# uc-vision/torch-darktable

Hardware: AMD Instinct MI355X
Metric: megapixels/sec full ISP (debayer->denoise->tonemap) 12MP RGGB (higher is better)
Workload: dtype f32; 1 GPU; 12 MP full pipeline (RCD -> Wiener log-L sigma=0.075 K=32 ov=4 -> bilateral sigma_s=2 sigma_r=0.2 detail=0.4 -> metrics -> Reinhard gamma=0.75 intensity=2 light_adapt=1 -> u8), batch 8 per GPU; width=4096, height=3072, streams_per_gpu=3, storage=f16, arithmetic=f32, chain=lab, issue=eager launches, denoiser=Wiener (the reference has no nlmeans / wavelet denoiser)

## Files before the change

### torch-darktable_amd/csrc/bilateral.hip

```cpp
#include <stdlib.h>

#include "tdk_color.h"

#ifdef TDK_BIL_TIMING
__device__ unsigned long long g_bil_phase_cycles[16];
#define BIL_MARK(k) do { if (threadIdx.x == 0 && blockIdx.x == 1000) { const unsigned long long t_ = clock64(); atomicAdd(&g_bil_phase_cycles[k], t_ - bil_t0); bil_t0 = t_; } } while (0)
extern "C" __attribute__((visibility("default"))) int tdk_debug_bilateral_phase_cycles(unsigned long long* out16, int reset) {
  if (hipMemcpyFromSymbol(out16, HIP_SYMBOL(g_bil_phase_cycles), sizeof(unsigned long long) * 16) != hipSuccess) return -1;
  if (reset) { unsigned long long z[16] = {}; if (hipMemcpyToSymbol(HIP_SYMBOL(g_bil_phase_cycles), z, sizeof z) != hipSuccess) return -1; }
  return 0;
}
#else
#define BIL_MARK(k)
#endif

namespace {

struct GridDims {
  int sx, sy, sz;
};

GridDims compute_grid_size(int width, int height, float sigma_s, float sigma_r) {
  float ss = sigma_s;
  if (ss < 0.5f) ss = 0.5f;
  const float L_range = 1.0f;
  auto clampf_h = [](float v, float lo, float hi) { return fminf(fmaxf(v, lo), hi); };
  const float gx = clampf_h(roundf((float)width / ss), 4.0f, 3000.0f);
  const float gy = clampf_h(roundf((float)height / ss), 4.0f, 3000.0f);
  const float gz = clampf_h(roundf(L_range / sigma_r), 4.0f, 50.0f);
  const float s_s = fmaxf((float)height / gy, (float)width / gx);
  const float s_r = L_range / gz;
  GridDims d;
  d.sx = (int)ceilf((float)width / s_s) + 1;
  d.sy = (int)ceilf((float)height / s_s) + 1;
  d.sz = (int)ceilf(L_range / s_r) + 1;
  return d;
}

struct Sample {
  int ix, iy, iz;
  float fx, fy, fz;
};

__device__ __forceinline__ Sample make_sample(int x, int y, float L, GridDims d, float sigma_s, float sigma_r) {
  const float gx = clampf((float)x / sigma_s, 0.0f, (float)(d.sx - 1));
  const float gy = clampf((float)y / sigma_s, 0.0f, (float)(d.sy - 1));
  const float gz = clampf(L / sigma_r, 0.0f, (float)(d.sz - 1));
  Sample s;
  s.ix = min((int)gx, d.sx - 2);
  s.iy = min((int)gy, d.sy - 2);
  s.iz = min((int)gz, d.sz - 2);
  s.fx = gx - (float)s.ix;
  s.fy = gy - (float)s.iy;
  s.fz = gz - (float)s.iz;
  return s;
}

__device__ __forceinline__ float axis_weight(int p, float sigma_s, int size, int cell) {
  const float g = clampf((float)p / sigma_s, 0.0f, (float)(size - 1));
  const int ib = min((int)g, size - 2);
  const float f = g - (float)ib;
  return (ib == cell) ? (1.0f - f) : ((ib == cell - 1) ? f : -1.0f);
}

template <typename T, int MAXC>
__global__ __launch_bounds__(256) void splat_gather_kernel(const T* __restrict__ lum, float* __restrict__ grid, int width, int height, GridDims d,
                                                           float sigma_s, float sigma_r) {
  extern __shared__ float colacc[];
  const int cx = blockIdx.x * 32 + (threadIdx.x & 31), cy = blockIdx.y * 8 + (threadIdx.x >> 5);
  const int tid = threadIdx.x;
  for (int z = 0; z < d.sz; z++) colacc[z * 256 + tid] = 0.0f;
  if (cx >= d.sx || cy >= d.sy) return;
  const float contrib = 1.0f / (sigma_s * sigma_s);
  const int x_lo = max(0, (int)floorf(sigma_s * (float)(cx - 1)) - 1);
  const int x_hi = (cx == d.sx - 1) ? width - 1 : min(width - 1, (int)ceilf(sigma_s * (float)(cx + 1)) + 1);
  const int y_lo = max(0, (int)floorf(sigma_s * (float)(cy - 1)) - 1);
  const int y_hi = (cy == d.sy - 1) ? height - 1 : min(height - 1, (int)ceilf(sigma_s * (float)(cy + 1)) + 1);

  auto deposit = [&](int x, int y, float wxy) {
    const float L = ld(lum, (size_t)y * width + x);
    const float gz = clampf(L / sigma_r, 0.0f, (float)(d.sz - 1));
    const int iz = min((int)gz, d.sz - 2);
    const float fz = gz - (float)iz;
    colacc[iz * 256 + tid] += wxy * (1.0f - fz) * contrib;
    colacc[(iz + 1) * 256 + tid] += wxy * fz * contrib;
  };

  if (x_hi - x_lo + 1 <= MAXC) {
    float wxs[MAXC];
#pragma unroll
    for (int k = 0; k < MAXC; k++) wxs[k] = (x_lo + k <= x_hi) ? axis_weight(x_lo + k, sigma_s, d.sx, cx) : -1.0f;
    for (int y = y_lo; y <= y_hi; y++) {
      const float wy = axis_weight(y, sigma_s, d.sy, cy);
      if (!(wy > 0.0f)) continue;
#pragma unroll
      for (int k = 0; k < MAXC; k++)
        if (wxs[k] > 0.0f) deposit(x_lo + k, y, wxs[k] * wy);
    }
  } else {
    for (int y = y_lo; y <= y_hi; y++) {
      const float wy = axis_weight(y, sigma_s, d.sy, cy);
      if (!(wy > 0.0f)) continue;
      for (int x = x_lo; x <= x_hi; x++) {
        const float wx = axis_weight(x, sigma_s, d.sx, cx);
        if (wx > 0.0f) deposit(x, y, wx * wy);
      }
    }
  }
  const size_t plane = (size_t)d.sx * d.sy;
  float* g = grid + (size_t)cy * d.sx + cx;
  for (int z = 0; z < d.sz; z++) g[z * plane] = colacc[z * 256 + tid];
}

constexpr int BTW = 64, BTH = 16;
constexpr int BLW = BTW + 4, BLH = BTH + 4;

__global__ __launch_bounds__(256) void blur_xy_kernel(const float* __restrict__ gin, float* __restrict__ gout, GridDims d) {
  __shared__ float a[BLH][BLW + 1];
  __shared__ float b[BLH][BTW + 1];
  const int x0 = blockIdx.x * BTW, y0 = blockIdx.y * BTH, z = blockIdx.z;
  const float* src = gin + (size_t)z * d.sx * d.sy;
  float* dst = gout + (size_t)z * d.sx * d.sy;
  for (int i = threadIdx.x; i < BLW * BLH; i += 256) {
    const int r = i / BLW, c = i - r * BLW;
    const int gx = x0 - 2 + c, gy = y0 - 2 + r;
    a[r][c] = (gx >= 0 && gy >= 0 && gx < d.sx && gy < d.sy) ? src[(size_t)gy * d.sx + gx] : 0.0f;
  }
  __syncthreads();
  const float w0 = 6.0f / 16.0f, w1 = 4.0f / 16.0f, w2 = 1.0f / 16.0f;
  for (int i = threadIdx.x; i < BTW * BLH; i += 256) {
    const int r = i / BTW, c = i - r * BTW;
    const float* p = &a[r][c + 2];
    const int gy = y0 - 2 + r;
    b[r][c] = (gy >= 0 && gy < d.sy) ? (p[0] * w0 + w1 * (p[1] + p[-1]) + w2 * (p[2] + p[-2])) : 0.0f;
  }
  __syncthreads();
  for (int i = threadIdx.x; i < BTW * BTH; i += 256) {
    const int r = i / BTW, c = i - r * BTW;
    const int gx = x0 + c, gy = y0 + r;
    if (gx < d.sx && gy < d.sy)
      dst[(size_t)gy * d.sx + gx] = b[r + 2][c] * w0 + w1 * (b[r + 3][c] + b[r + 1][c]) + w2 * (b[r + 4][c] + b[r][c]);
  }
}

__global__ __launch_bounds__(256) void blur_z_kernel(const float* __restrict__ gin, float* __restrict__ gout, GridDims d) {
  const size_t plane = (size_t)d.sx * d.sy;
  const size_t i = (size_t)blockIdx.x * 256 + threadIdx.x;
  if (i >= plane) return;
  const float w1 = 4.0f / 16.0f, w2 = 2.0f / 16.0f;
  float m2 = 0.0f, m1 = 0.0f;
  float c0 = gin[i];
  float p1 = (d.sz > 1) ? gin[i + plane] : 0.0f;
  for (int z = 0; z < d.sz; z++) {
    const float p2 = (z + 2 < d.sz) ? gin[i + (size_t)(z + 2) * plane] : 0.0f;
    gout[i + (size_t)z * plane] = w1 * (p1 - m1) + w2 * (p2 - m2);
    m2 = m1; m1 = c0; c0 = p1; p1 = p2;
  }
}

template <typename T>
__global__ __launch_bounds__(256) void slice_kernel(const T* __restrict__ lum, const float* __restrict__ grid, T* __restrict__ out, int width,
                                                    int height, GridDims d, float sigma_s, float sigma_r, float detail) {
  const int64_t n = (int64_t)width * height;
  const float norm = -detail * sigma_r * 4.0f;
  const size_t oy = d.sx, oz = (size_t)d.sx * d.sy;
  for (int64_t i = (int64_t)blockIdx.x * 256 + threadIdx.x; i < n; i += (int64_t)gridDim.x * 256) {
    const int y = (int)(i / width), x = (int)(i - (int64_t)y * width);
    const float L = ld(lum, (size_t)i);
    const Sample s = make_sample(x, y, L, d, sigma_s, sigma_r);
    const float ax = 1.0f - s.fx, ay = 1.0f - s.fy, az = 1.0f - s.fz, bx = s.fx, by = s.fy, bz = s.fz;
    const float* g = grid + s.ix + oy * s.iy + oz * s.iz;
    const float Ldiff = g[0] * ax * ay * az + g[1] * bx * ay * az + g[oy] * ax * by * az + g[oy + 1] * bx * by * az + g[oz] * ax * ay * bz +
                        g[oz + 1] * bx * ay * bz + g[oz + oy] * ax * by * bz + g[oz + oy + 1] * bx * by * bz;
    st(out, (size_t)i, fmaxf(0.0f, L + norm * Ldiff));
  }
}

template <typename T, bool LOG, int VEC>
__global__ __launch_bounds__(256) void slice_modify_kernel(const float* __restrict__ lum, const float* __restrict__ grid, const T* __restrict__ rgb,
                                                           T* __restrict__ out, int width, int height, GridDims d, float sigma_s, float sigma_r,
                                                           float detail) {
  const int64_t n = (int64_t)width * height / VEC;
  const float norm = -detail * sigma_r * 4.0f;
  const size_t oy = d.sx, oz = (size_t)d.sx * d.sy;
  for (int64_t gi = (int64_t)blockIdx.x * 256 + threadIdx.x; gi < n; gi += (int64_t)gridDim.x * 256) {
    const int64_t i0 = gi * VEC;
    const int y = (int)(i0 / width), x0 = (int)(i0 - (int64_t)y * width);
    float v[3 * VEC], Lv[VEC];
    if constexpr (VEC == 4) {
      rgb4_io<T>::load(rgb, (size_t)gi, v);
      s4_io<float>::load(lum, (size_t)gi, Lv);
    } else {
      v[0] = ld(rgb, (size_t)i0 * 3); v[1] = ld(rgb, (size_t)i0 * 3 + 1); v[2] = ld(rgb, (size_t)i0 * 3 + 2);
      Lv[0] = lum[i0];
    }
#pragma unroll
    for (int k = 0; k < VEC; k++) {
      const float L = Lv[k];
      const Sample s = make_sample(x0 + k, y, L, d, sigma_s, sigma_r);
      const float ax = 1.0f - s.fx, ay = 1.0f - s.fy, az = 1.0f - s.fz, bx = s.fx, by = s.fy, bz = s.fz;
      const float* g = grid + s.ix + oy * s.iy + oz * s.iz;
      const float Ldiff = g[0] * ax * ay * az + g[1] * bx * ay * az + g[oy] * ax * by * az + g[oy + 1] * bx * by * az + g[oz] * ax * ay * bz +
                          g[oz + 1] * bx * ay * bz + g[oz + oy] * ax * by * bz + g[oz + oy + 1] * bx * by * bz;
      const float Lnew = fmaxf(0.0f, L + norm * Ldiff);
      const f3 c = mk3(v[3 * k], v[3 * k + 1], v[3 * k + 2]);
      const f3 r = LOG ? cA::modify_log_luminance(c, Lnew) : cA::modify_luminance(c, Lnew);
      v[3 * k] = r.x; v[3 * k + 1] = r.y; v[3 * k + 2] = r.z;
    }
    if constexpr (VEC == 4) rgb4_io<T>::store(out, (size_t)gi, v);
    else { st(out, (size_t)i0 * 3, v[0]); st(out, (size_t)i0 * 3 + 1, v[1]); st(out, (size_t)i0 * 3 + 2, v[2]); }
  }
}

template <typename T>
__global__ __launch_bounds__(256) void slice_lab_kernel(const float* __restrict__ lum, const float* __restrict__ grid, const float* __restrict__ ab,
                                                        T* __restrict__ out, int width, int height, GridDims d, float sigma_s, float sigma_r, float detail) {
  const int64_t n = (int64_t)width * height;
  const float norm = -detail * sigma_r * 4.0f;
  const size_t oy = d.sx, oz = (size_t)d.sx * d.sy;
  for (int64_t i = (int64_t)blockIdx.x * 256 + threadIdx.x; i < n; i += (int64_t)gridDim.x * 256) {
    const int y = (int)(i / width), x = (int)(i - (int64_t)y * width);
    const float L = lum[i];
    const Sample s = make_sample(x, y, L, d, sigma_s, sigma_r);
    const float ax = 1.0f - s.fx, ay = 1.0f - s.fy, az = 1.0f - s.fz, bx = s.fx, by = s.fy, bz = s.fz;
    const float* g = grid + s.ix + oy * s.iy + oz * s.iz;
    const float Ldiff = g[0] * ax * ay * az + g[1] * bx * ay * az + g[oy] * ax * by * az + g[oy + 1] * bx * by * az + g[oz] * ax * ay * bz +
                        g[oz + 1] * bx * ay * bz + g[oz + oy] * ax * by * bz + g[oz + oy + 1] * bx * by * bz;
    const float Lnew = fmaxf(0.0f, L + norm * Ldiff);
    const f3 r = clip3(cA::lab_to_rgb(mk3(fmaxf(0.0f, fminf(1.0f, Lnew)), ab[2 * i], ab[2 * i + 1])));
    st(out, (size_t)i * 3, r.x); st(out, (size_t)i * 3 + 1, r.y); st(out, (size_t)i * 3 + 2, r.z);
  }
}

constexpr int FTW = 64, FTH = 32, FNT = 512;
constexpr int TAB_HDR = 4;
constexpr int TAB_W = 8;

struct AxisTile {
  int c_lo;
  int nc;
  int p_lo;
  int np;
};

__host__ __device__ inline AxisTile axis_tile(int p0, int tile, int size_px, int size_cells, float sigma_s) {
  const int p1 = ((p0 + tile < size_px) ? p0 + tile : size_px) - 1;
  const float top = (float)(size_cells - 1);
  const float g0 = fminf(fmaxf((float)p0 / sigma_s, 0.0f), top), g1 = fminf(fmaxf((float)p1 / sigma_s, 0.0f), top);
  const int c0 = ((int)g0 < size_cells - 2) ? (int)g0 : size_cells - 2;
  const int c1 = (((int)g1 < size_cells - 2) ? (int)g1 : size_cells - 2) + 1;
  AxisTile t;
  t.c_lo = c0 - 2;
  t.nc = c1 - c0 + 5;
  const int lo = (int)floorf(sigma_s * (float)(t.c_lo - 1)) - 1;
  const int hi = (int)ceilf(sigma_s * (float)(c1 + 3)) + 1;
  t.p_lo = lo > 0 ? lo : 0;
  t.np = ((hi < size_px - 1) ? hi : size_px - 1) - t.p_lo + 1;
  return t;
}

struct TileLds {
  int rs;
  int plane;
  int usize;
  int lw, lh;
  int ncx, ncy;
  int hx, hy;
  float inv_lw, inv_qw, inv_rs, inv_ncy;
  float rc_r, contrib, norm;
};

__host__ __device__ inline int win_lo(int p0, int halo) { return p0 > halo ? p0 - halo : 0; }
__host__ __device__ inline int win_np(int lo, int lp, int size_px) { return lo + lp < size_px ? lp : size_px - lo; }

__host__ __device__ inline int tab_rec(int lp, int nc) { return TAB_HDR + lp + nc * (1 + TAB_W); }

__global__ __launch_bounds__(64) void bilateral_axis_tables_kernel(int* __restrict__ tab, int width, int height, GridDims d, float sigma_s, int tiles_x,
                                                                  TileLds L) {
  __shared__ int s_nmax;
  const bool is_x = (int)blockIdx.x < tiles_x;
  const int ti = is_x ? (int)blockIdx.x : (int)blockIdx.x - tiles_x;
  const int size_px = is_x ? width : height, size_cells = is_x ? d.sx : d.sy, tile = is_x ? FTW : FTH;
  const int lp = is_x ? L.lw : L.lh, ncm = is_x ? L.ncx : L.ncy, halo = is_x ? L.hx : L.hy;
  int* rec = tab + (is_x ? ti * tab_rec(L.lw, L.ncx) : tiles_x * tab_rec(L.lw, L.ncx) + ti * tab_rec(L.lh, L.ncy));
  const AxisTile t = axis_tile(ti * tile, tile, size_px, size_cells, sigma_s);
  const int p_lo = win_lo(ti * tile, halo), np = win_np(p_lo, lp, size_px);
  float* gs = reinterpret_cast<float*>(rec + TAB_HDR);
  int* start = rec + TAB_HDR + lp;
  float* wt = reinterpret_cast<float*>(start + ncm);
  const int lane = threadIdx.x;
  if (lane == 0) s_nmax = 1;
  __syncthreads();
  for (int i = lane; i < np; i += 64) gs[i] = clampf((float)(p_lo + i) / sigma_s, 0.0f, (float)(size_cells - 1));
  for (int l = lane; l < t.nc; l += 64) {
    const int cell = t.c_lo + l;
    int first = -1;
    if (cell >= 0 && cell < size_cells) {
      const int a = max(p_lo, (int)floorf(sigma_s * (float)(cell - 1)) - 1);
      const int b = min(p_lo + np - 1, (int)ceilf(sigma_s * (float)(cell + 1)) + 1);
      int k0 = -1, k1 = -1;
      for (int p = a; p <= b; p++)
        if (axis_weight(p, sigma_s, size_cells, cell) > 0.0f) { if (k0 < 0) k0 = p; k1 = p; }
      first = k0 < 0 ? a : k0;
      if (k0 >= 0) atomicMax(&s_nmax, k1 - k0 + 1);
    }
    start[l] = first;
  }
  __syncthreads();
  const int nmax = min(s_nmax, min(TAB_W, np));
  for (int l = lane; l < t.nc; l += 64) {
    const int cell = t.c_lo + l;
    int first = start[l];
    if (first >= 0) {
      first = min(first, p_lo + np - nmax);
      start[l] = first - p_lo;
    }
    for (int k = 0; k < TAB_W; k++) {
      float w = 0.0f;
      if (first >= 0 && k < nmax) w = fmaxf(axis_weight(first + k, sigma_s, size_cells, cell), 0.0f);
      wt[k * ncm + l] = w;
    }
  }
  if (lane == 0) { rec[0] = t.c_lo; rec[1] = t.nc; rec[2] = nmax; }
}

__device__ __forceinline__ int fast_div(int i, float inv) { return (int)(((float)i + 0.5f) * inv); }

__device__ __forceinline__ void lds_barrier() {
  __builtin_amdgcn_fence(__ATOMIC_RELEASE, "workgroup", "local");
  __builtin_amdgcn_s_barrier();
  __builtin_amdgcn_fence(__ATOMIC_ACQUIRE, "workgroup", "local");
}

#define TDK_BT_FAST 0
namespace bt_exact {
#include "tdk_bilateral_tile.h"
}
#undef TDK_BT_FAST
#define TDK_BT_FAST 1
#pragma clang fp contract(fast)
namespace bt_fast {
#include "tdk_bilateral_tile.h"
}
#pragma clang fp contract(off)
#undef TDK_BT_FAST

constexpr size_t FUSED_LDS_LIMIT = 80 * 1024;

static bool plan_tiles(int width, int height, const GridDims& d, float sigma_s, float sigma_r, float detail, TileLds* L, size_t* lds_bytes) {
  if (!(sigma_s >= 1.0f && sigma_s <= 4.0f)) return false;
  if ((float)(width - 1) / sigma_s > (float)(d.sx - 1) || (float)(height - 1) / sigma_s > (float)(d.sy - 1)) return false;
  int ncx = 0, ncy = 0, hx = 0, hy = 0, lw = 0, lh = 0;
  for (int x0 = 0; x0 < width; x0 += FTW) {
    const AxisTile t = axis_tile(x0, FTW, width, d.sx, sigma_s);
    ncx = t.nc > ncx ? t.nc : ncx; hx = x0 - t.p_lo > hx ? x0 - t.p_lo : hx;
  }
  hx = (hx + 3) & ~3;
  for (int x0 = 0; x0 < width; x0 += FTW) {
    const AxisTile t = axis_tile(x0, FTW, width, d.sx, sigma_s);
    const int n = t.p_lo + t.np - win_lo(x0, hx);
    lw = n > lw ? n : lw;
  }
  lw = (lw + 3) & ~3;
  for (int y0 = 0; y0 < height; y0 += FTH) {
    const AxisTile t = axis_tile(y0, FTH, height, d.sy, sigma_s);
    ncy = t.nc > ncy ? t.nc : ncy; hy = y0 - t.p_lo > hy ? y0 - t.p_lo : hy;
  }
  for (int y0 = 0; y0 < height; y0 += FTH) {
    const AxisTile t = axis_tile(y0, FTH, height, d.sy, sigma_s);
    const int n = t.p_lo + t.np - win_lo(y0, hy);
    lh = n > lh ? n : lh;
  }
  L->rs = ncx | 1;
  L->plane = (int)tdk_align_up((size_t)L->rs * ncy, 64);
  const int lt = lw * lh + (ncx + ncy) * (1 + TAB_W), bt = d.sz * L->plane;
  L->usize = (int)tdk_align_up((size_t)(lt > bt ? lt : bt), 64);
  L->lw = lw; L->lh = lh;
  L->ncx = ncx; L->ncy = ncy;
  L->hx = hx; L->hy = hy;
  L->inv_lw = 1.0f / (float)lw; L->inv_qw = 1.0f / (float)(lw / 4); L->inv_rs = 1.0f / (float)L->rs; L->inv_ncy = 1.0f / (float)ncy;
  L->rc_r = 1.0f / sigma_r; L->contrib = 1.0f / (sigma_s * sigma_s); L->norm = -detail * sigma_r * 4.0f;
  *lds_bytes = ((size_t)d.sz * L->plane + L->usize + (size_t)lw + (size_t)lh) * sizeof(float);
  if (lw > 2 * FNT || lh > 2 * FNT || ncx * (1 + TAB_W) > 2 * FNT || ncy * (1 + TAB_W) > 2 * FNT) return false;
  return *lds_bytes <= FUSED_LDS_LIMIT;
}

static size_t tile_table_bytes(int width, int height, float sigma_s, float sigma_r) {
  const GridDims d = compute_grid_size(width, height, sigma_s, sigma_r);
  TileLds L;
  size_t lds_bytes = 0;
  if (!plan_tiles(width, height, d, sigma_s, sigma_r, 0.0f, &L, &lds_bytes)) return 0;
  const size_t words = (size_t)tdk_div_up(width, FTW) * tab_rec(L.lw, L.ncx) + (size_t)tdk_div_up(height, FTH) * tab_rec(L.lh, L.ncy);
  return tdk_align_up(words * sizeof(int), 256);
}

static int build_tables(int* tab, int width, int height, const GridDims& d, float sigma_s, const TileLds& L, hipStream_t s) {
  const int tiles_x = tdk_div_up(width, FTW), tiles_y = tdk_div_up(height, FTH);
  TDK_LAUNCH("tdk_bilateral(tables)", bilateral_axis_tables_kernel, dim3(tiles_x + tiles_y), dim3(64), 0, s, tab, width, height, d, sigma_s, tiles_x, L);
  return TDK_OK;
}

template <typename TL, typename T, int MODE>
int launch_tiles(const TL* lum, const T* rgb, T* out, int* tab, int width, int height, const GridDims& d, float sigma_s, float sigma_r, float detail,
                 const TileLds& L, size_t lds_bytes, bool vec, bool prepared, hipStream_t s) {
  const int tiles_x = tdk_div_up(width, FTW), tiles_y = tdk_div_up(height, FTH), ntiles = tiles_x * tiles_y;
  const dim3 grid(8 * tdk_div_up(ntiles, 8));
#ifdef TDK_EXPERIMENTS
  if (const char* e = getenv("TDK_BIL_LDS_PAD")) lds_bytes += (size_t)atoi(e);
#endif
  if (!prepared) {
    const int rc = build_tables(tab, width, height, d, sigma_s, L, s);
    if (rc != TDK_OK) return rc;
  }
#define TDK_BT(NS, VECV)                                                                                                                          \
  do {                                                                                                                                            \
    TDK_MAX_LDS_ONCE((NS::bilateral_tile_kernel<TL, T, MODE, VECV>), "tdk_bilateral(hipFuncSetAttribute)");                                       \
    TDK_LAUNCH("tdk_bilateral(tiles)", (NS::bilateral_tile_kernel<TL, T, MODE, VECV>), grid, dim3(FNT), lds_bytes, s, lum, rgb, out, tab, width, height, d, \
               sigma_r, tiles_x, ntiles, L);                                                                                                      \
  } while (0)
  if constexpr (MODE == 3) { if (vec) TDK_BT(bt_fast, 4); else TDK_BT(bt_fast, 1); }
  else { if (vec) TDK_BT(bt_exact, 4); else TDK_BT(bt_exact, 1); }
#undef TDK_BT
  return TDK_OK;
}

static size_t grid_floats(const GridDims& d) { return tdk_align_up((size_t)d.sx * d.sy * d.sz, 64); }
static size_t plane_workspace_bytes(const GridDims& d, size_t tables) { return tables + tdk_align_up(2 * grid_floats(d) * sizeof(float), 256); }
static size_t rgb_workspace_bytes(const GridDims& d, int width, int height, size_t tables) {
  return tables + tdk_align_up((2 * grid_floats(d) + (size_t)width * height) * sizeof(float), 256);
}

template <typename T>
int build_grid(const T* in, float* grid, float* tmp, int width, int height, const GridDims& d, float sigma_s, float sigma_r, hipStream_t s) {
  const size_t splat_lds = (size_t)d.sz * 256 * sizeof(float);
  const dim3 sgrid(tdk_div_up(d.sx, 32), tdk_div_up(d.sy, 8));
  if (2.0f * sigma_s + 5.0f <= 10.0f) {
    TDK_MAX_LDS_ONCE((splat_gather_kernel<T, 10>), "tdk_bilateral(hipFuncSetAttribute)");
    TDK_LAUNCH("tdk_bilateral(splat)", (splat_gather_kernel<T, 10>), sgrid, dim3(256), splat_lds, s, in, grid, width, height, d, sigma_s, sigma_r);
  } else {
    TDK_MAX_LDS_ONCE((splat_gather_kernel<T, 24>), "tdk_bilateral(hipFuncSetAttribute)");
    TDK_LAUNCH("tdk_bilateral(splat)", (splat_gather_kernel<T, 24>), sgrid, dim3(256), splat_lds, s, in, grid, width, height, d, sigma_s, sigma_r);
  }
  TDK_LAUNCH("tdk_bilateral(blur_xy)", blur_xy_kernel, dim3(tdk_div_up(d.sx, BTW), tdk_div_up(d.sy, BTH), d.sz), dim3(256), 0, s, grid, tmp, d);
  TDK_LAUNCH("tdk_bilateral(blur_z)", blur_z_kernel, dim3((unsigned)tdk_div_up64((int64_t)d.sx * d.sy, 256)), dim3(256), 0, s, tmp, grid, d);
  return TDK_OK;
}

inline unsigned stream_blocks(int64_t npix) {
  int64_t b = tdk_div_up64(npix, 256);
  return (unsigned)(b > 4096 ? 4096 : (b < 1 ? 1 : b));
}

template <typename T>
int launch(const void* lum_in, void* lum_out, void* workspace, int width, int height, float sigma_s, float sigma_r, float detail, unsigned flags, hipStream_t s) {
  const GridDims d = compute_grid_size(width, height, sigma_s, sigma_r);
  const size_t tables = tile_table_bytes(width, height, sigma_s, sigma_r);
  int* tab = reinterpret_cast<int*>(workspace);
  float* grid = reinterpret_cast<float*>(reinterpret_cast<char*>(workspace) + tables);
  float* tmp = grid + grid_floats(d);
  const T* in = reinterpret_cast<const T*>(lum_in);
  TileLds L;
  size_t lds_bytes = 0;
  const bool tiles = !(flags & TDK_BILATERAL_GENERAL_PATH) && lum_in != lum_out
                     && plan_tiles(width, height, d, sigma_s, sigma_r, detail, &L, &lds_bytes);
  if (tiles) {
    const bool vec = (width % 4) == 0 && tdk_aligned(lum_in, 16) && tdk_aligned(lum_out, 16);
    return launch_tiles<T, T, 0>(in, nullptr, reinterpret_cast<T*>(lum_out), tab, width, height, d, sigma_s, sigma_r, detail, L, lds_bytes, vec,
                                 (flags & TDK_BILATERAL_PREPARED) != 0, s);
  }
  const int rc = build_grid<T>(in, grid, tmp, width, height, d, sigma_s, sigma_r, s);
  if (rc != TDK_OK) return rc;
  TDK_LAUNCH("tdk_bilateral(slice)", slice_kernel<T>, dim3(stream_blocks((int64_t)width * height)), dim3(256), 0, s, in, grid, reinterpret_cast<T*>(lum_out),
             width, height, d, sigma_s, sigma_r, detail);
  return TDK_OK;
}

template <typename T>
int launch_rgb(const void* rgb_in, void* rgb_out, void* workspace, int width, int height, float sigma_s, float sigma_r, float detail, int log_mode, float eps,
               int dtype, unsigned flags, hipStream_t s, const float* lum_in = nullptr) {
  const GridDims d = compute_grid_size(width, height, sigma_s, sigma_r);
  const size_t tables = tile_table_bytes(width, height, sigma_s, sigma_r);
  int* tab = reinterpret_cast<int*>(workspace);
  float* grid = reinterpret_cast<float*>(reinterpret_cast<char*>(workspace) + tables);
  float* tmp = grid + grid_floats(d);
  const float* plane = lum_in;
  int rc = TDK_OK;
  if (!plane) {
    float* mine = tmp + grid_floats(d);
    rc = tdk_compute_luminance(rgb_in, mine, (int64_t)width * height, log_mode, eps, dtype, TDK_F32, reinterpret_cast<tdk_stream_t>(s));
    if (rc != TDK_OK) return rc;
    plane = mine;
  }
  const bool vec = (width % 4) == 0 && tdk_aligned(rgb_in, 16) && tdk_aligned(rgb_out, 16) && tdk_aligned(plane, 16);
  TileLds L;
  size_t lds_bytes = 0;
  if (!(flags & TDK_BILATERAL_GENERAL_PATH) && plan_tiles(width, height, d, sigma_s, sigma_r, detail, &L, &lds_bytes)) {
    const bool prepared = (flags & TDK_BILATERAL_PREPARED) != 0;
    if (log_mode) return launch_tiles<float, T, 2>(plane, reinterpret_cast<const T*>(rgb_in), reinterpret_cast<T*>(rgb_out), tab, width, height, d, sigma_s, sigma_r, detail, L, lds_bytes, vec, prepared, s);
    return launch_tiles<float, T, 1>(plane, reinterpret_cast<const T*>(rgb_in), reinterpret_cast<T*>(rgb_out), tab, width, height, d, sigma_s, sigma_r, detail, L, lds_bytes, vec, prepared, s);
  }
  rc = build_grid<float>(plane, grid, tmp, width, height, d, sigma_s, sigma_r, s);
  if (rc != TDK_OK) return rc;
  const unsigned blocks = stream_blocks((int64_t)width * height / (vec ? 4 : 1));
  const T* rin = reinterpret_cast<const T*>(rgb_in);
  T* rout = reinterpret_cast<T*>(rgb_out);
#define TDK_SM(LOGV, VECV) \
  TDK_LAUNCH("tdk_bilateral(slice+modify)", (slice_modify_kernel<T, LOGV, VECV>), dim3(blocks), dim3(256), 0, s, plane, grid, rin, rout, width, height, d, \
             sigma_s, sigma_r, detail)
  if (log_mode) { if (vec) TDK_SM(true, 4); else TDK_SM(true, 1); }
  else { if (vec) TDK_SM(false, 4); else TDK_SM(false, 1); }
#undef TDK_SM
  return TDK_OK;
}

template <typename T>
int launch_lab(const float* lum, const float* ab, void* rgb_out, void* workspace, int width, int height, float sigma_s, float sigma_r, float detail, unsigned flags,
               hipStream_t s) {
  const GridDims d = compute_grid_size(width, height, sigma_s, sigma_r);
  const size_t tables = tile_table_bytes(width, height, sigma_s, sigma_r);
  int* tab = reinterpret_cast<int*>(workspace);
  float* grid = reinterpret_cast<float*>(reinterpret_cast<char*>(workspace) + tables);
  float* tmp = grid + grid_floats(d);
  TileLds L;
  size_t lds_bytes = 0;
  if (!(flags & TDK_BILATERAL_GENERAL_PATH) && plan_tiles(width, height, d, sigma_s, sigma_r, detail, &L, &lds_bytes)) {
    const bool vec = (width % 4) == 0 && tdk_aligned(rgb_out, 16) && tdk_aligned(lum, 16) && tdk_aligned(ab, 16);
    return launch_tiles<float, T, 3>(lum, reinterpret_cast<const T*>(ab), reinterpret_cast<T*>(rgb_out), tab, width, height, d, sigma_s, sigma_r, detail, L, lds_bytes,
                                     vec, (flags & TDK_BILATERAL_PREPARED) != 0, s);
  }
  const int rc = build_grid<float>(lum, grid, tmp, width, height, d, sigma_s, sigma_r, s);
  if (rc != TDK_OK) return rc;
  TDK_LAUNCH("tdk_bilateral(slice+lab)", slice_lab_kernel<T>, dim3(stream_blocks((int64_t)width * height)), dim3(256), 0, s, lum, grid, ab, reinterpret_cast<T*>(rgb_out),
             width, height, d, sigma_s, sigma_r, detail);
  return TDK_OK;
}

}

TDK_EXPORT int tdk_bilateral_lab(const float* lum_in, const float* ab_in, void* rgb_out, void* workspace, int width, int height, float sigma_s, float sigma_r,
                                 float detail, int out_dtype, unsigned flags, tdk_stream_t stream) {
  TDK_REQUIRE(lum_in && ab_in && rgb_out && workspace, "tdk_bilateral_lab: null pointer");
  TDK_REQUIRE(width > 0 && height > 0, "Invalid dimensions");
  TDK_REQUIRE(sigma_s > 0.0f && sigma_r > 0.0f, "tdk_bilateral_lab: sigmas must be positive");
  TDK_REQUIRE((flags & ~(TDK_BILATERAL_PREPARED | TDK_BILATERAL_GENERAL_PATH)) == 0, "tdk_bilateral_lab: unknown flags 0x%x", flags);
  TDK_DISPATCH_DTYPE(out_dtype, T, return launch_lab<T>(lum_in, ab_in, rgb_out, workspace, width, height, sigma_s, sigma_r, detail, flags, tdk_stream(stream)));
  return TDK_OK;
}

TDK_EXPORT int tdk_bilateral_grid_size(int width, int height, float sigma_s, float sigma_r, int size_xyz[3]) {
  TDK_REQUIRE(width > 0 && height > 0 && sigma_r > 0.0f && size_xyz, "tdk_bilateral_grid_size: invalid arguments");
  const GridDims d = compute_grid_size(width, height, sigma_s, sigma_r);
  size_xyz[0] = d.sx; size_xyz[1] = d.sy; size_xyz[2] = d.sz;
  return TDK_OK;
}

TDK_EXPORT size_t tdk_bilateral_workspace_bytes(int width, int height, float sigma_s, float sigma_r) {
  if (width <= 0 || height <= 0 || !(sigma_r > 0.0f)) return 0;
  const GridDims d = compute_grid_size(width, height, sigma_s, sigma_r);
  return plane_workspace_bytes(d, tile_table_bytes(width, height, sigma_s, sigma_r));
}

TDK_EXPORT size_t tdk_bilateral_rgb_workspace_bytes(int width, int height, float sigma_s, float sigma_r) {
  if (width <= 0 || height <= 0 || !(sigma_r > 0.0f)) return 0;
  const GridDims d = compute_grid_size(width, height, sigma_s, sigma_r);
  return rgb_workspace_bytes(d, width, height, tile_table_bytes(width, height, sigma_s, sigma_r));
}

TDK_EXPORT int tdk_bilateral_prepare(void* workspace, int width, int height, float sigma_s, float sigma_r, tdk_stream_t stream) {
  TDK_REQUIRE(workspace, "tdk_bilateral_prepare: null pointer");
  TDK_REQUIRE(width > 0 && height > 0, "Invalid dimensions");
  TDK_REQUIRE(sigma_s > 0.0f && sigma_r > 0.0f, "tdk_bilateral_prepare: sigmas must be positive");
  const GridDims d = compute_grid_size(width, height, sigma_s, sigma_r);
  TileLds L;
  size_t lds_bytes = 0;
  if (!plan_tiles(width, height, d, sigma_s, sigma_r, 0.0f, &L, &lds_bytes)) return TDK_OK;
  return build_tables(reinterpret_cast<int*>(workspace), width, height, d, sigma_s, L, tdk_stream(stream));
}

TDK_EXPORT int tdk_bilateral_ex(const void* lum_in, void* lum_out, void* workspace, int width, int height, float sigma_s, float sigma_r,
                                float detail, int dtype, unsigned flags, tdk_stream_t stream) {
  TDK_REQUIRE(lum_in && lum_out && workspace, "tdk_bilateral: null pointer");
  TDK_REQUIRE(width > 0 && height > 0, "Invalid dimensions");
  TDK_REQUIRE(sigma_s > 0.0f && sigma_r > 0.0f, "tdk_bilateral: sigmas must be positive");
  TDK_REQUIRE((flags & ~(TDK_BILATERAL_PREPARED | TDK_BILATERAL_GENERAL_PATH)) == 0, "tdk_bilateral: unknown flags 0x%x", flags);
  TDK_DISPATCH_DTYPE(dtype, T, return launch<T>(lum_in, lum_out, workspace, width, height, sigma_s, sigma_r, detail, flags, tdk_stream(stream)));
  return TDK_OK;
}

TDK_EXPORT int tdk_bilateral(const void* lum_in, void* lum_out, void* workspace, int width, int height, float sigma_s, float sigma_r,
                             float detail, int dtype, tdk_stream_t stream) {
  return tdk_bilateral_ex(lum_in, lum_out, workspace, width, height, sigma_s, sigma_r, detail, dtype, 0u, stream);
}

TDK_EXPORT int tdk_bilateral_rgb_ex(const void* rgb_in, const float* lum_in, void* rgb_out, void* workspace, int width, int height, float sigma_s,
                                    float sigma_r, float detail, int log_mode, float eps, int dtype, unsigned flags, tdk_stream_t stream) {
  TDK_REQUIRE(rgb_in && rgb_out && workspace, "tdk_bilateral_rgb: null pointer");
  TDK_REQUIRE(width > 0 && height > 0, "Invalid dimensions");
  TDK_REQUIRE(sigma_s > 0.0f && sigma_r > 0.0f, "tdk_bilateral_rgb: sigmas must be positive");
  TDK_REQUIRE(!log_mode || eps > 0.0f, "Epsilon must be positive");
  TDK_REQUIRE((flags & ~(TDK_BILATERAL_PREPARED | TDK_BILATERAL_GENERAL_PATH)) == 0, "tdk_bilateral_rgb: unknown flags 0x%x", flags);
  TDK_DISPATCH_DTYPE(dtype, T, return launch_rgb<T>(rgb_in, rgb_out, workspace, width, height, sigma_s, sigma_r, detail, log_mode, eps, dtype, flags, tdk_stream(stream), lum_in));
  return TDK_OK;
}

TDK_EXPORT int tdk_bilateral_rgb(const void* rgb_in, void* rgb_out, void* workspace, int width, int height, float sigma_s, float sigma_r, float detail,
                                 int log_mode, float eps, int dtype, tdk_stream_t stream) {
  return tdk_bilateral_rgb_ex(rgb_in, nullptr, rgb_out, workspace, width, height, sigma_s, sigma_r, detail, log_mode, eps, dtype, 0u, stream);
}

TDK_EXPORT int tdk_bilateral_rgb_lum(const void* rgb_in, const float* lum_in, void* rgb_out, void* workspace, int width, int height, float sigma_s,
                                     float sigma_r, float detail, int log_mode, float eps, int dtype, tdk_stream_t stream) {
  TDK_REQUIRE(lum_in, "tdk_bilateral_rgb_lum: null pointer");
  return tdk_bilateral_rgb_ex(rgb_in, lum_in, rgb_out, workspace, width, height, sigma_s, sigma_r, detail, log_mode, eps, dtype, 0u, stream);
}
```

### torch-darktable_amd/csrc/tdk_bilateral_tile.h

```cpp

template <int NX>
__device__ __forceinline__ void splat_column(float* __restrict__ acc, const float* __restrict__ urow, const float* __restrict__ wxp, int wxs_stride,
                                             const float* __restrict__ wyp, int wys_stride, int nmy, int LWS, int PS, int sz, float contrib) {
  float wxs[NX];
#pragma unroll
  for (int k = 0; k < NX; k++) wxs[k] = wxp[k * wxs_stride];
  for (int j = 0; j < nmy; j++, urow += LWS) {
    const float wy = wyp[j * wys_stride];
    float gzv[NX];
#pragma unroll
    for (int k = 0; k < NX; k++) gzv[k] = urow[k];
#pragma unroll
    for (int k = 0; k < NX; k++) {
      const float wxy = wxs[k] * wy;
      const float gz = gzv[k];
      const int iz = min((int)gz, sz - 2);
      const float fz = gz - (float)iz;
      float* p0 = acc + iz * PS;
      const float a0 = p0[0], a1 = p0[PS];
#if TDK_BT_FAST
      const float wc = wxy * contrib;
      p0[0] = __builtin_fmaf(wc, 1.0f - fz, a0);
      p0[PS] = __builtin_fmaf(wc, fz, a1);
#else
      p0[0] = a0 + wxy * (1.0f - fz) * contrib;
      p0[PS] = a1 + wxy * fz * contrib;
#endif
    }
  }
}

template <int N>
__device__ __forceinline__ void sample_gz(const float (&v)[N], float (&g)[N], float sigma_r, float rc_r, float ztop) {
#if TDK_BT_FAST
#pragma unroll
  for (int k = 0; k < N; k++) g[k] = clampf(v[k] * rc_r, 0.0f, ztop);
  return;
#endif
  float hi = fabsf(v[0]);
  float lo = (v[0] == 0.0f) ? 1.0f : hi;
#pragma unroll
  for (int k = 1; k < N; k++) {
    const float a = fabsf(v[k]);
    hi = fmaxf(hi, a);
    lo = fminf(lo, (v[k] == 0.0f) ? 1.0f : a);
  }
  bool safe = lo >= 0x1p-40f && hi <= 0x1p40f && sigma_r >= 0x1p-20f && sigma_r <= 0x1p20f;
#pragma unroll
  for (int k = 0; k < N; k++) safe = safe && (v[k] == v[k]);
  if (__builtin_expect(__builtin_amdgcn_ballot_w64(!safe) != 0, 0)) {
#pragma unroll
    for (int k = 0; k < N; k++) g[k] = clampf(v[k] / sigma_r, 0.0f, ztop);
    return;
  }
#pragma unroll
  for (int k = 0; k < N; k++) {
    const float q = v[k] * rc_r;
    const float r = __builtin_fmaf(-q, sigma_r, v[k]);
    g[k] = clampf(__builtin_fmaf(r, rc_r, q), 0.0f, ztop);
  }
}

template <typename TL, typename T, int MODE, int VEC>
#ifndef TDK_BIL_WPE
#define TDK_BIL_WPE 8
#endif
__global__ __launch_bounds__(FNT) __attribute__((amdgpu_waves_per_eu(TDK_BIL_WPE, TDK_BIL_WPE))) void bilateral_tile_kernel(
    const TL* __restrict__ lum, const T* __restrict__ rgb, T* __restrict__ out, const int* __restrict__ tab, int width, int height, GridDims d,
    float sigma_r, int tiles_x, int ntiles, TileLds L) {
  extern __shared__ float smem[];
#ifdef TDK_BIL_TIMING
  unsigned long long bil_t0 = clock64();
#endif
  float* A = smem;
  float* U = A + d.sz * L.plane;
  float* gxs = U + L.usize;
  float* gys = gxs + L.lw;
  int* TX = reinterpret_cast<int*>(U + L.lw * L.lh);
  int* TY = TX + L.ncx * (1 + TAB_W);

  const int chunk = gridDim.x >> 3;
  const int tile = (blockIdx.x & 7) * chunk + (blockIdx.x >> 3);
  if (tile >= ntiles) return;
  const int tyi = tile / tiles_x, txi = tile - tyi * tiles_x;
  const int x0 = txi * FTW, y0 = tyi * FTH;
  const int recx = tab_rec(L.lw, L.ncx), recy = tab_rec(L.lh, L.ncy);
  const int* rx = tab + txi * recx;
  const int* ry = tab + tiles_x * recx + tyi * recy;
  const int px_lo = win_lo(x0, L.hx), py_lo = win_lo(y0, L.hy);
  const int npx = win_np(px_lo, L.lw, width), npy = win_np(py_lo, L.lh, height);
  const int tid = threadIdx.x;
  const int PS = L.plane, RS = L.rs, LWS = L.lw;
  const float ztop = (float)(d.sz - 1), rc_r = L.rc_r;

  {
    auto copy2 = [&](int* dst, const int* from, int n) {
      if (tid < n) dst[tid] = from[tid];
      if (tid + FNT < n) dst[tid + FNT] = from[tid + FNT];
    };
    auto copy_records = [&]() {
      copy2(reinterpret_cast<int*>(gxs), rx + TAB_HDR, L.lw);
      copy2(reinterpret_cast<int*>(gys), ry + TAB_HDR, L.lh);
      copy2(TX, rx + TAB_HDR + L.lw, L.ncx * (1 + TAB_W));
      copy2(TY, ry + TAB_HDR + L.lh, L.ncy * (1 + TAB_W));
    };
    const TL* src = lum + (size_t)py_lo * width + px_lo;
    if constexpr (VEC == 4) {
      const int qw = L.lw >> 2, total = qw * npy;
      constexpr int NB = 2;
      for (int base = tid; base - tid < total; base += NB * FNT) {
        float v[NB][4];
        int at[NB];
#pragma unroll
        for (int k = 0; k < NB; k++) {
          const int q = base + k * FNT;
          const int r = fast_div(q, L.inv_qw), c = (q - r * qw) * 4;
          at[k] = (q < total && c < npx) ? r * LWS + c : -1;
          if (at[k] >= 0) s4_io<TL>::load(src + (size_t)r * width + c, 0, v[k]);
        }
        if (base == tid) copy_records();
#pragma unroll
        for (int k = 0; k < NB; k++) {
          if (at[k] >= 0) {
            float g[4];
            sample_gz<4>(v[k], g, sigma_r, rc_r, ztop);
            *reinterpret_cast<float4*>(U + at[k]) = make_float4(g[0], g[1], g[2], g[3]);
          }
        }
      }
    } else {
      const int total = LWS * npy;
      constexpr int NB = 7;
      for (int base = tid; base - tid < total; base += NB * FNT) {
        float v[NB];
        bool on[NB];
#pragma unroll
        for (int k = 0; k < NB; k++) {
          const int i = base + k * FNT;
          const int r = fast_div(i, L.inv_lw), c = i - r * LWS;
          on[k] = i < total && c < npx;
          v[k] = on[k] ? ld(src, (size_t)r * width + c) : 0.0f;
        }
        if (base == tid) copy_records();
        float g[NB];
        sample_gz<NB>(v, g, sigma_r, rc_r, ztop);
#pragma unroll
        for (int k = 0; k < NB; k++)
          if (on[k]) U[base + k * FNT] = g[k];
      }
    }
  }
  AxisTile ax, ay;
  ax.c_lo = rx[0]; ax.nc = rx[1]; ay.c_lo = ry[0]; ay.nc = ry[1];
  const int nmx = rx[2], nmy = ry[2];
  BIL_MARK(8);
  lds_barrier();
  BIL_MARK(0);

  const float contrib = L.contrib;
  {
    const int ncol = RS * ay.nc;
    const float* WX = reinterpret_cast<const float*>(TX + L.ncx);
    const float* WY = reinterpret_cast<const float*>(TY + L.ncy);
    for (int c = tid; c < ncol; c += FNT) {
      const int ly = fast_div(c, L.inv_rs), lx = c - ly * RS;
      if (lx >= ax.nc) continue;
      const int xa = TX[lx], ya = TY[ly];
      float* acc = A + c;
      for (int z = 0; z < d.sz; z++) acc[z * PS] = 0.0f;
      if (xa < 0 || ya < 0) continue;
      const float* urow = U + ya * LWS + xa;
      const float* wxp = WX + lx;
      const float* wyp = WY + ly;
      switch (nmx) {
        case 1: splat_column<1>(acc, urow, wxp, L.ncx, wyp, L.ncy, nmy, LWS, PS, d.sz, contrib); break;
        case 2: splat_column<2>(acc, urow, wxp, L.ncx, wyp, L.ncy, nmy, LWS, PS, d.sz, contrib); break;
        case 3: splat_column<3>(acc, urow, wxp, L.ncx, wyp, L.ncy, nmy, LWS, PS, d.sz, contrib); break;
        case 4: splat_column<4>(acc, urow, wxp, L.ncx, wyp, L.ncy, nmy, LWS, PS, d.sz, contrib); break;
        case 5: splat_column<5>(acc, urow, wxp, L.ncx, wyp, L.ncy, nmy, LWS, PS, d.sz, contrib); break;
        case 6: splat_column<6>(acc, urow, wxp, L.ncx, wyp, L.ncy, nmy, LWS, PS, d.sz, contrib); break;
        case 7: splat_column<7>(acc, urow, wxp, L.ncx, wyp, L.ncy, nmy, LWS, PS, d.sz, contrib); break;
        default: splat_column<8>(acc, urow, wxp, L.ncx, wyp, L.ncy, nmy, LWS, PS, d.sz, contrib); break;
      }
    }
  }
  lds_barrier();
  BIL_MARK(1);

  const float w0 = 6.0f / 16.0f, w1 = 4.0f / 16.0f, w2 = 1.0f / 16.0f;
  {
    constexpr int CH = 13;
    for (int row = tid; row < d.sz * L.ncy; row += FNT) {
      const int z = fast_div(row, L.inv_ncy), ly = row - z * L.ncy;
      if (ly >= ay.nc) continue;
      const float* p = A + z * PS + ly * RS;
      float* q = U + z * PS + ly * RS;
      float m2 = 0.0f, m1 = 0.0f, c0 = p[0], p1 = p[1];
      for (int lx0 = 0; lx0 < ax.nc; lx0 += CH) {
        float nx[CH];
#pragma unroll
        for (int k = 0; k < CH; k++) nx[k] = (lx0 + k + 2 < ax.nc) ? p[lx0 + k + 2] : 0.0f;
#pragma unroll
        for (int k = 0; k < CH; k++) {
          if (lx0 + k < ax.nc) q[lx0 + k] = c0 * w0 + w1 * (p1 + m1) + w2 * (nx[k] + m2);
          m2 = m1; m1 = c0; c0 = p1; p1 = nx[k];
        }
      }
    }
  }
  lds_barrier();
  BIL_MARK(2);
  {
    constexpr int CH = 11;
    for (int cc = tid; cc < d.sz * RS; cc += FNT) {
      const int z = fast_div(cc, L.inv_rs), lx = cc - z * RS;
      if (lx >= ax.nc) continue;
      const float* p = U + z * PS + lx;
      float* q = A + z * PS + lx;
      float m2 = 0.0f, m1 = 0.0f, c0 = p[0], p1 = p[RS];
      for (int ly0 = 0; ly0 < ay.nc; ly0 += CH) {
        float nx[CH];
#pragma unroll
        for (int k = 0; k < CH; k++) nx[k] = (ly0 + k + 2 < ay.nc) ? p[(ly0 + k + 2) * RS] : 0.0f;
#pragma unroll
        for (int k = 0; k < CH; k++) {
          if (ly0 + k < ay.nc) q[(ly0 + k) * RS] = c0 * w0 + w1 * (p1 + m1) + w2 * (nx[k] + m2);
          m2 = m1; m1 = c0; c0 = p1; p1 = nx[k];
        }
      }
    }
  }
  lds_barrier();
  BIL_MARK(3);
  {
    const float v1 = 4.0f / 16.0f, v2 = 2.0f / 16.0f;
    constexpr int ZR = 8;
    for (int c = tid; c < RS * ay.nc; c += FNT) {
      float* p = A + c;
      if (d.sz <= ZR) {
        float v[ZR + 4];
        v[0] = v[1] = 0.0f;
#pragma unroll
        for (int z = 0; z < ZR + 2; z++) v[z + 2] = (z < d.sz) ? p[z * PS] : 0.0f;
#pragma unroll
        for (int z = 0; z < ZR; z++)
          if (z < d.sz) p[z * PS] = v1 * (v[z + 3] - v[z + 1]) + v2 * (v[z + 4] - v[z]);
      } else {
        float m2 = 0.0f, m1 = 0.0f, c0 = p[0];
        float p1 = (d.sz > 1) ? p[PS] : 0.0f;
        for (int z = 0; z < d.sz; z++) {
          const float p2 = (z + 2 < d.sz) ? p[(z + 2) * PS] : 0.0f;
          p[z * PS] = v1 * (p1 - m1) + v2 * (p2 - m2);
          m2 = m1; m1 = c0; c0 = p1; p1 = p2;
        }
      }
    }
  }
  lds_barrier();
  BIL_MARK(4);

  const float norm = L.norm;
  constexpr int GW = FTW / VEC;
  for (int g = tid; g < GW * FTH; g += FNT) {
    const int py = g / GW, y = y0 + py, x = x0 + (g - py * GW) * VEC;
    if (x >= width || y >= height) continue;
    const size_t i0 = (size_t)y * width + x;
    float Lv[VEC], o[MODE == 0 ? VEC : 3 * VEC], c2[MODE == 3 ? 2 * VEC : 1];
    if constexpr (VEC == 4) {
      s4_io<TL>::load(lum, i0 >> 2, Lv);
      if constexpr (MODE == 3) {
        const float* ab = reinterpret_cast<const float*>(rgb);
        s4_io<float>::load(ab, i0 >> 1, c2);
        s4_io<float>::load(ab, (i0 >> 1) + 1, c2 + 4);
      } else if constexpr (MODE != 0) {
        rgb4_io<T>::load(rgb, i0 >> 2, o);
      }
    } else {
      Lv[0] = ld(lum, i0);
      if constexpr (MODE == 3) { const float* ab = reinterpret_cast<const float*>(rgb); c2[0] = ab[2 * i0]; c2[1] = ab[2 * i0 + 1]; }
      else if constexpr (MODE != 0) { o[0] = ld(rgb, i0 * 3); o[1] = ld(rgb, i0 * 3 + 1); o[2] = ld(rgb, i0 * 3 + 2); }
    }
    const float gy = gys[y - py_lo];
    const int iy = min((int)gy, d.sy - 2);
    const float by = gy - (float)iy, ayw = 1.0f - by;
    const float* grow = A + (iy - ay.c_lo) * RS - ax.c_lo;
    float gzv[VEC];
    sample_gz<VEC>(Lv, gzv, sigma_r, rc_r, ztop);
#pragma unroll
    for (int k = 0; k < VEC; k++) {
      const float Lp = Lv[k];
      const float gx = gxs[x + k - px_lo];
      const int ix = min((int)gx, d.sx - 2);
      const float bx = gx - (float)ix, axw = 1.0f - bx;
      const float gz = gzv[k];
      const int iz = min((int)gz, d.sz - 2);
      const float bz = gz - (float)iz, azw = 1.0f - bz;
      const int oy = RS, oz = PS;
      const float* gp = grow + iz * PS + ix;
#if TDK_BT_FAST
      auto lerp2 = [](float a, float b, float t) { return __builtin_fmaf(t, b - a, a); };
      const float z0 = lerp2(lerp2(gp[0], gp[1], bx), lerp2(gp[oy], gp[oy + 1], bx), by);
      const float z1 = lerp2(lerp2(gp[oz], gp[oz + 1], bx), lerp2(gp[oz + oy], gp[oz + oy + 1], bx), by);
      const float Ldiff = lerp2(z0, z1, bz);
      (void)axw; (void)ayw; (void)azw;
#else
      const float Ldiff = gp[0] * axw * ayw * azw + gp[1] * bx * ayw * azw + gp[oy] * axw * by * azw + gp[oy + 1] * bx * by * azw +
                          gp[oz] * axw * ayw * bz + gp[oz + 1] * bx * ayw * bz + gp[oz + oy] * axw * by * bz + gp[oz + oy + 1] * bx * by * bz;
#endif
      const float Lnew = fmaxf(0.0f, Lp + norm * Ldiff);
      if constexpr (MODE == 0) {
        o[k] = Lnew;
      } else if constexpr (MODE == 3) {
        const f3 r = clip3(cA::lab_to_rgb(mk3(fmaxf(0.0f, fminf(1.0f, Lnew)), c2[2 * k], c2[2 * k + 1])));
        o[3 * k] = r.x; o[3 * k + 1] = r.y; o[3 * k + 2] = r.z;
      } else {
        const f3 c = mk3(o[3 * k], o[3 * k + 1], o[3 * k + 2]);
        const f3 r = (MODE == 2) ? cA::modify_log_luminance(c, Lnew) : cA::modify_luminance(c, Lnew);
        o[3 * k] = r.x; o[3 * k + 1] = r.y; o[3 * k + 2] = r.z;
      }
    }
    if constexpr (MODE == 0) {
      if constexpr (VEC == 4) s4_io<T>::store(out, i0 >> 2, o);
      else st(out, i0, o[0]);
    } else {
      if constexpr (VEC == 4) rgb4_io<T>::store(out, i0 >> 2, o);
      else { st(out, i0 * 3, o[0]); st(out, i0 * 3 + 1, o[1]); st(out, i0 * 3 + 2, o[2]); }
    }
  }
  BIL_MARK(5);
}
```

Baseline: 31590 MP/s.

## Specialize bilateral tile kernel on grid depth and pad LDS blur rows

Adds a template parameter for the bilateral grid's z-depth (5–12) so the splat, blur and gradient loops unroll fully with compile-time trip counts. It also pads the LDS cell layout to multiples of the blur chunk sizes, which removes the per-element bounds checks in the x and y blur passes. The padded layout is used only when it keeps the same number of tiles resident per CU and keeps all padded reads inside the allocation. In exchange there are more kernel instantiations and possibly more LDS per tile, and the padded cells are computed redundantly.

```diff
diff --git a/torch-darktable_amd/csrc/bilateral.hip b/torch-darktable_amd/csrc/bilateral.hip
--- a/torch-darktable_amd/csrc/bilateral.hip
+++ b/torch-darktable_amd/csrc/bilateral.hip
@@ -235,6 +235,7 @@
 constexpr int FTW = 64, FTH = 32, FNT = 512;
 constexpr int TAB_HDR = 4;
 constexpr int TAB_W = 8;
+constexpr int BX_CH = 13, BY_CH = 7;
 
 struct AxisTile {
   int c_lo;
@@ -265,6 +266,7 @@
   int usize;
   int lw, lh;
   int ncx, ncy;
+  int ncxp, ncyp;
   int hx, hy;
   float inv_lw, inv_qw, inv_rs, inv_ncy;
   float rc_r, contrib, norm;
@@ -345,7 +347,13 @@
 #pragma clang fp contract(off)
 #undef TDK_BT_FAST
 
-constexpr size_t FUSED_LDS_LIMIT = 80 * 1024;
+constexpr size_t CU_LDS = 160 * 1024;
+constexpr size_t LDS_GRANULE = 512;
+constexpr size_t FUSED_LDS_LIMIT = CU_LDS / 2;
+static size_t tiles_per_cu(size_t lds) {
+  const size_t n = CU_LDS / tdk_align_up(lds, LDS_GRANULE);
+  return n < 4 ? n : 4;
+}
 
 static bool plan_tiles(int width, int height, const GridDims& d, float sigma_s, float sigma_r, float detail, TileLds* L, size_t* lds_bytes) {
   if (!(sigma_s >= 1.0f && sigma_s <= 4.0f)) return false;
@@ -371,16 +379,32 @@
     const int n = t.p_lo + t.np - win_lo(y0, hy);
     lh = n > lh ? n : lh;
   }
-  L->rs = ncx | 1;
-  L->plane = (int)tdk_align_up((size_t)L->rs * ncy, 64);
-  const int lt = lw * lh + (ncx + ncy) * (1 + TAB_W), bt = d.sz * L->plane;
-  L->usize = (int)tdk_align_up((size_t)(lt > bt ? lt : bt), 64);
+  const int lt = lw * lh + (ncx + ncy) * (1 + TAB_W);
+  auto layout = [&](int rs, int rows, TileLds* o) {
+    o->rs = rs;
+    o->plane = (int)tdk_align_up((size_t)rs * rows, 64);
+    const int bt = d.sz * o->plane;
+    o->usize = (int)tdk_align_up((size_t)(lt > bt ? lt : bt), 64);
+    return ((size_t)d.sz * o->plane + o->usize + (size_t)lw + (size_t)lh) * sizeof(float);
+  };
+  *lds_bytes = layout(ncx | 1, ncy, L);
+  L->ncxp = L->ncyp = 0;
+  {
+    const int ncxp = (int)tdk_align_up(ncx, BX_CH), ncyp = (int)tdk_align_up(ncy, BY_CH);
+    TileLds P;
+    const size_t bytes = layout(ncxp | 1, ncyp, &P);
+    const bool reads_inside = (size_t)(d.sz - 1) * P.plane + (size_t)(ncyp + 2) * P.rs <= (size_t)P.usize + lw + lh;
+    if (reads_inside && tiles_per_cu(bytes) >= tiles_per_cu(*lds_bytes)) {
+      L->rs = P.rs; L->plane = P.plane; L->usize = P.usize;
+      L->ncxp = ncxp; L->ncyp = ncyp;
+      *lds_bytes = bytes;
+    }
+  }
   L->lw = lw; L->lh = lh;
   L->ncx = ncx; L->ncy = ncy;
   L->hx = hx; L->hy = hy;
   L->inv_lw = 1.0f / (float)lw; L->inv_qw = 1.0f / (float)(lw / 4); L->inv_rs = 1.0f / (float)L->rs; L->inv_ncy = 1.0f / (float)ncy;
   L->rc_r = 1.0f / sigma_r; L->contrib = 1.0f / (sigma_s * sigma_s); L->norm = -detail * sigma_r * 4.0f;
-  *lds_bytes = ((size_t)d.sz * L->plane + L->usize + (size_t)lw + (size_t)lh) * sizeof(float);
   if (lw > 2 * FNT || lh > 2 * FNT || ncx * (1 + TAB_W) > 2 * FNT || ncy * (1 + TAB_W) > 2 * FNT) return false;
   return *lds_bytes <= FUSED_LDS_LIMIT;
 }
@@ -412,14 +436,30 @@
     const int rc = build_tables(tab, width, height, d, sigma_s, L, s);
     if (rc != TDK_OK) return rc;
   }
-#define TDK_BT(NS, VECV)                                                                                                                          \
+#define TDK_BT(NS, VECV, SZV)                                                                                                                     \
   do {                                                                                                                                            \
-    TDK_MAX_LDS_ONCE((NS::bilateral_tile_kernel<TL, T, MODE, VECV>), "tdk_bilateral(hipFuncSetAttribute)");                                       \
-    TDK_LAUNCH("tdk_bilateral(tiles)", (NS::bilateral_tile_kernel<TL, T, MODE, VECV>), grid, dim3(FNT), lds_bytes, s, lum, rgb, out, tab, width, height, d, \
-               sigma_r, tiles_x, ntiles, L);                                                                                                      \
+    TDK_MAX_LDS_ONCE((NS::bilateral_tile_kernel<TL, T, MODE, VECV, SZV>), "tdk_bilateral(hipFuncSetAttribute)");                                  \
+    TDK_LAUNCH("tdk_bilateral(tiles)", (NS::bilateral_tile_kernel<TL, T, MODE, VECV, SZV>), grid, dim3(FNT), lds_bytes, s, lum, rgb, out, tab, width, \
+               height, d, sigma_r, tiles_x, ntiles, L);                                                                                           \
   } while (0)
-  if constexpr (MODE == 3) { if (vec) TDK_BT(bt_fast, 4); else TDK_BT(bt_fast, 1); }
-  else { if (vec) TDK_BT(bt_exact, 4); else TDK_BT(bt_exact, 1); }
+  if constexpr (MODE == 3) {
+    if (vec && L.ncxp > 0) {
+      switch (d.sz) {
+        case 5: TDK_BT(bt_fast, 4, 5); return TDK_OK;
+        case 6: TDK_BT(bt_fast, 4, 6); return TDK_OK;
+        case 7: TDK_BT(bt_fast, 4, 7); return TDK_OK;
+        case 8: TDK_BT(bt_fast, 4, 8); return TDK_OK;
+        case 9: TDK_BT(bt_fast, 4, 9); return TDK_OK;
+        case 10: TDK_BT(bt_fast, 4, 10); return TDK_OK;
+        case 11: TDK_BT(bt_fast, 4, 11); return TDK_OK;
+        case 12: TDK_BT(bt_fast, 4, 12); return TDK_OK;
+        default: break;
+      }
+    }
+    if (vec) TDK_BT(bt_fast, 4, 0); else TDK_BT(bt_fast, 1, 0);
+  } else {
+    if (vec) TDK_BT(bt_exact, 4, 0); else TDK_BT(bt_exact, 1, 0);
+  }
 #undef TDK_BT
   return TDK_OK;
 }
diff --git a/torch-darktable_amd/csrc/tdk_bilateral_tile.h b/torch-darktable_amd/csrc/tdk_bilateral_tile.h
--- a/torch-darktable_amd/csrc/tdk_bilateral_tile.h
+++ b/torch-darktable_amd/csrc/tdk_bilateral_tile.h
@@ -1,10 +1,11 @@
 
-template <int NX>
+template <int NX, int NY = 0>
 __device__ __forceinline__ void splat_column(float* __restrict__ acc, const float* __restrict__ urow, const float* __restrict__ wxp, int wxs_stride,
                                              const float* __restrict__ wyp, int wys_stride, int nmy, int LWS, int PS, int sz, float contrib) {
   float wxs[NX];
 #pragma unroll
   for (int k = 0; k < NX; k++) wxs[k] = wxp[k * wxs_stride];
+  if constexpr (NY > 0) nmy = NY;
   for (int j = 0; j < nmy; j++, urow += LWS) {
     const float wy = wyp[j * wys_stride];
     float gzv[NX];
@@ -61,7 +62,7 @@
   }
 }
 
-template <typename TL, typename T, int MODE, int VEC>
+template <typename TL, typename T, int MODE, int VEC, int SZC>
 #ifndef TDK_BIL_WPE
 #define TDK_BIL_WPE 8
 #endif
@@ -72,8 +73,9 @@
 #ifdef TDK_BIL_TIMING
   unsigned long long bil_t0 = clock64();
 #endif
+  const int sz = SZC > 0 ? SZC : d.sz;
   float* A = smem;
-  float* U = A + d.sz * L.plane;
+  float* U = A + sz * L.plane;
   float* gxs = U + L.usize;
   float* gys = gxs + L.lw;
   int* TX = reinterpret_cast<int*>(U + L.lw * L.lh);
@@ -91,7 +93,7 @@
   const int npx = win_np(px_lo, L.lw, width), npy = win_np(py_lo, L.lh, height);
   const int tid = threadIdx.x;
   const int PS = L.plane, RS = L.rs, LWS = L.lw;
-  const float ztop = (float)(d.sz - 1), rc_r = L.rc_r;
+  const float ztop = (float)(sz - 1), rc_r = L.rc_r;
 
   {
     auto copy2 = [&](int* dst, const int* from, int n) {
@@ -167,28 +169,51 @@
       if (lx >= ax.nc) continue;
       const int xa = TX[lx], ya = TY[ly];
       float* acc = A + c;
-      for (int z = 0; z < d.sz; z++) acc[z * PS] = 0.0f;
+      for (int z = 0; z < sz; z++) acc[z * PS] = 0.0f;
       if (xa < 0 || ya < 0) continue;
       const float* urow = U + ya * LWS + xa;
       const float* wxp = WX + lx;
       const float* wyp = WY + ly;
+#define TDK_SPLAT(NXV)                                                                                                         \
+  if (SZC > 0 && nmy == NXV) splat_column<NXV, NXV>(acc, urow, wxp, L.ncx, wyp, L.ncy, nmy, LWS, PS, sz, contrib);             \
+  else splat_column<NXV>(acc, urow, wxp, L.ncx, wyp, L.ncy, nmy, LWS, PS, sz, contrib);                                        \
+  break
       switch (nmx) {
-        case 1: splat_column<1>(acc, urow, wxp, L.ncx, wyp, L.ncy, nmy, LWS, PS, d.sz, contrib); break;
-        case 2: splat_column<2>(acc, urow, wxp, L.ncx, wyp, L.ncy, nmy, LWS, PS, d.sz, contrib); break;
-        case 3: splat_column<3>(acc, urow, wxp, L.ncx, wyp, L.ncy, nmy, LWS, PS, d.sz, contrib); break;
-        case 4: splat_column<4>(acc, urow, wxp, L.ncx, wyp, L.ncy, nmy, LWS, PS, d.sz, contrib); break;
-        case 5: splat_column<5>(acc, urow, wxp, L.ncx, wyp, L.ncy, nmy, LWS, PS, d.sz, contrib); break;
-        case 6: splat_column<6>(acc, urow, wxp, L.ncx, wyp, L.ncy, nmy, LWS, PS, d.sz, contrib); break;
-        case 7: splat_column<7>(acc, urow, wxp, L.ncx, wyp, L.ncy, nmy, LWS, PS, d.sz, contrib); break;
-        default: splat_column<8>(acc, urow, wxp, L.ncx, wyp, L.ncy, nmy, LWS, PS, d.sz, contrib); break;
-      }
+        case 1: TDK_SPLAT(1);
+        case 2: TDK_SPLAT(2);
+        case 3: TDK_SPLAT(3);
+        case 4: TDK_SPLAT(4);
+        case 5: TDK_SPLAT(5);
+        case 6: TDK_SPLAT(6);
+        case 7: TDK_SPLAT(7);
+        default: TDK_SPLAT(8);
+      }
+#undef TDK_SPLAT
     }
   }
   lds_barrier();
   BIL_MARK(1);
 
   const float w0 = 6.0f / 16.0f, w1 = 4.0f / 16.0f, w2 = 1.0f / 16.0f;
-  {
+  if constexpr (SZC > 0) {
+    constexpr int CH = BX_CH;
+    for (int row = tid; row < SZC * L.ncy; row += FNT) {
+      const int z = fast_div(row, L.inv_ncy), ly = row - z * L.ncy;
+      const float* p = A + z * PS + ly * RS;
+      float* q = U + z * PS + ly * RS;
+      float m2 = 0.0f, m1 = 0.0f, c0 = p[0], p1 = p[1];
+      for (int lx0 = 0; lx0 < L.ncxp; lx0 += CH) {
+        float nx[CH];
+#pragma unroll
+        for (int k = 0; k < CH; k++) nx[k] = p[lx0 + k + 2];
+#pragma unroll
+        for (int k = 0; k < CH; k++) {
+          q[lx0 + k] = c0 * w0 + w1 * (p1 + m1) + w2 * (nx[k] + m2);
+          m2 = m1; m1 = c0; c0 = p1; p1 = nx[k];
+        }
+      }
+    }
+  } else {
     constexpr int CH = 13;
     for (int row = tid; row < d.sz * L.ncy; row += FNT) {
       const int z = fast_div(row, L.inv_ncy), ly = row - z * L.ncy;
@@ -210,7 +235,25 @@
   }
   lds_barrier();
   BIL_MARK(2);
-  {
+  if constexpr (SZC > 0) {
+    constexpr int CH = BY_CH;
+    for (int cc = tid; cc < SZC * RS; cc += FNT) {
+      const int z = fast_div(cc, L.inv_rs), lx = cc - z * RS;
+      const float* p = U + z * PS + lx;
+      float* q = A + z * PS + lx;
+      float m2 = 0.0f, m1 = 0.0f, c0 = p[0], p1 = p[RS];
+      for (int ly0 = 0; ly0 < L.ncyp; ly0 += CH) {
+        float nx[CH];
+#pragma unroll
+        for (int k = 0; k < CH; k++) nx[k] = p[(ly0 + k + 2) * RS];
+#pragma unroll
+        for (int k = 0; k < CH; k++) {
+          q[(ly0 + k) * RS] = c0 * w0 + w1 * (p1 + m1) + w2 * (nx[k] + m2);
+          m2 = m1; m1 = c0; c0 = p1; p1 = nx[k];
+        }
+      }
+    }
+  } else {
     constexpr int CH = 11;
     for (int cc = tid; cc < d.sz * RS; cc += FNT) {
       const int z = fast_div(cc, L.inv_rs), lx = cc - z * RS;
@@ -232,8 +275,18 @@
   }
   lds_barrier();
   BIL_MARK(3);
-  {
-    const float v1 = 4.0f / 16.0f, v2 = 2.0f / 16.0f;
+  const float v1 = 4.0f / 16.0f, v2 = 2.0f / 16.0f;
+  if constexpr (SZC > 0) {
+    for (int c = tid; c < RS * ay.nc; c += FNT) {
+      float* p = A + c;
+      float v[SZC + 4];
+      v[0] = v[1] = v[SZC + 2] = v[SZC + 3] = 0.0f;
+#pragma unroll
+      for (int z = 0; z < SZC; z++) v[z + 2] = p[z * PS];
+#pragma unroll
+      for (int z = 0; z < SZC; z++) p[z * PS] = v1 * (v[z + 3] - v[z + 1]) + v2 * (v[z + 4] - v[z]);
+    }
+  } else {
     constexpr int ZR = 8;
     for (int c = tid; c < RS * ay.nc; c += FNT) {
       float* p = A + c;
@@ -293,7 +346,7 @@
       const int ix = min((int)gx, d.sx - 2);
       const float bx = gx - (float)ix, axw = 1.0f - bx;
       const float gz = gzv[k];
-      const int iz = min((int)gz, d.sz - 2);
+      const int iz = min((int)gz, sz - 2);
       const float bz = gz - (float)iz, azw = 1.0f - bz;
       const int oy = RS, oz = PS;
       const float* gp = grow + iz * PS + ix;
```

After: 32930 MP/s, median of 6. 4.2% higher.
